# rust-av/grav1synth

Measured on AMD Instinct MI355X. Metric: diff Mpixels/s (luma pixels of frame pairs fully processed: flat-block finder + AR accumulation + block stats + ordered fold), higher is better.
Workload: dtype i8 x i8 -> i32 matrix-core products, i64 sums (exact integers) + f64 flat-block features

## Files before the change

### grav1synth_amd/csrc/engine.hip

```cpp
#include <hip/hip_runtime.h>

#include <algorithm>
#include <chrono>
#include <cmath>
#include <cstdio>
#include <cstring>
#include <atomic>
#include <condition_variable>
#include <deque>
#include <functional>
#include <map>
#include <mutex>
#include <string>
#include <thread>
#include <type_traits>
#include <utility>
#include <vector>

#include "../../include/g1s_diff.h"
#include "fold.h"
#include "frame_op.h"
#include "host_pool.h"
#include "kernels.hip.h"
#include "k1f.hip.h"
// ... 660 lines not shown
    rc = flush_pending();
    if (rc) return rc;
  }
  {
    std::unique_lock<std::mutex> lk(dm);
    cur = (si + 1) % kSlots;
    cv_free.wait(lk, [&] { return !slot_busy[cur]; });
  }
  trace_host("next slot free", cur);
  return G1S_OK;
}

int g1s_diff::plan_batch(int si) {
  Slot &sl = slots[si];
  BatchPlan &p = sl.plan;
  p.g = batch_geom(sl);
  p.wide = wide_ok(p.g, batch_far(sl));
  p.timed = timing;
  p.chain = timing && timing_chain;
  const g1s_sched::Schedule s = g1s_sched::schedule(switches(), {p.timed, device_latest, p.wide, batch, si, p.g.nplanes, last_back});
  if ((s.latest == Role::latest || s.latest == Role::latest2) && !ensure_latest_streams(ss)) return fail_hip("the device half's streams could not be created");
  const hipStream_t of[] = {ss.compute, ss.flat, ss.flat2, ss.copy, ss.upload, ss.latest, ss.latest2};
  p.table = of[(int)s.table], p.finder = of[(int)s.finder], p.accum = of[(int)s.accum], p.rest = of[(int)s.rest];
  p.latest = of[(int)s.latest], p.d2h = of[(int)s.d2h];
  p.back_now = s.back_now, p.after = s.after, p.host_waits = s.host_waits;
  sl.marks.n = 0, sl.marks.timed = p.timed && !p.chain, sl.marks.trace = trace && !p.timed;
  return G1S_OK;
}

int g1s_diff::flush_pending() {
  if (pending < 0) return G1S_OK;
  const int si = pending;
  pending = -1;
  return launch_back(si);
}

int g1s_diff::launch_front(int si) {
  Slot &sl = slots[si];
  const BatchPlan &p = sl.plan;
  const Geom &g = p.g;
  const uint32_t B = sl.count;
  const hipStream_t up = p.table, fstream = p.finder;
  const FrameTable ft{sl.d_planes};
  if (sl.async_in) {
    if (up != ss.upload) {
      if (!h2d_order) HIP_TRY(hipEventCreateWithFlags(&h2d_order.p, hipEventDisableTiming));
      HIP_TRY(hipEventRecord(h2d_order, ss.upload));
      HIP_TRY(hipStreamWaitEvent(up, h2d_order, 0));
    }
    sl.async_in = false;
  }
  sl.marks.mark_trace(up, "table H2D");
  HIP_TRY(hipMemcpyAsync(sl.d_planes, sl.h_planes, sizeof(FramePlanes) * B, hipMemcpyHostToDevice, up));
  sl.marks.mark_trace(up, "k_zero");
  {
    ZeroJob z{};
    int nz = 0;
    auto fill = [&](uint8_t *base, size_t off, size_t bytes) { z.ptr[nz] = reinterpret_cast<uint32_t *>(base + off), z.ndw[nz++] = (uint32_t)(bytes / 4); };
    fill(sl.d_records, 0, L.size * B);
    fill(sl.d_mu, lay.mu_count, lay.mu_only - lay.mu_count);
    fill(sl.d_mu, lay.mu_only, lay.mu_only_bytes);
    fill(sl.d_k1, lay.k1_count, lay.k1 - lay.k1_count);
    if (switches().wide && sl.d_wu) fill(sl.d_wu, lay.wu_lbad, lay.wu_lbad_bytes);
    hipLaunchKernelGGL(k_zero, dim3(256), dim3(256), 0, up, z);
  }
  sl.marks.mark_trace(up, nullptr);
  if (up != p.accum) {
    HIP_TRY(hipEventRecord(ss.table_done[si], up));
    HIP_TRY(hipStreamWaitEvent(p.accum, ss.table_done[si], 0));
    HIP_TRY(hipStreamWaitEvent(fstream, ss.table_done[si], 0));
  }
  if (p.after >= 0) HIP_TRY(hipStreamWaitEvent(fstream, ss.kernels_done[p.after], 0));
  if (p.timed) HIP_TRY(hipEventRecord(sl.ev[kEvStart], fstream));
  {
    const int literal_mode = flat_literal ? flat_literal : switches().k1_literal;
    const int force_literal = literal_mode ? 1 : 0;
    int32_t *mom = reinterpret_cast<int32_t *>(sl.d_k1 + lay.k1_moments);
    CertifyLists cl;
    cl.list = reinterpret_cast<uint32_t *>(sl.d_k1 + lay.k1_list);
    cl.count = reinterpret_cast<uint32_t *>(sl.d_k1 + lay.k1_count);
    cl.global = literal_mode == 0 ? 1 : 0;
    const char *k1_rows = getenv("G1S_K1_ROWS");
    const bool strips = g.fast_rows && g.W % kBlock == 0 && literal_mode == 0 && !(k1_rows && atoi(k1_rows) != 0);
    if (strips) {
      constexpr int kR2 = G1S_STRIP_ROWS2, kRif = G1S_STRIP_RIF;
      constexpr bool kNt = G1S_STRIP_NT != 0, kFold = G1S_STRIP_FOLD != 0;
      if (p.timed && !p.chain) HIP_TRY(hipEventRecord(sl.ev[kEvMomStart], fstream));
      const char *keep_e = getenv("G1S_K1_KEEP_MB");
      const size_t keep_bytes = (size_t)(keep_e ? std::max(atoi(keep_e), 0) : kStripKeepMB) << 20;
      const size_t keep = std::min<size_t>(keep_bytes / ((size_t)g.W * g.src_bps * g.H), B);
      const int nt_frames = kNt ? (int)(B - keep) : 0;
      const dim3 sg((strip_tiles<kR2>(g.nbw, g.nbh) + 3) / 4, B);
      sl.marks.mark(fstream, g.src_bps == 1 ? "k1_moments_strips<1>" : "k1_moments_strips<2>");
      if (g.src_bps == 1)
        hipLaunchKernelGGL((k1_moments_strips<1, kR2, kRif, kNt, kFold>), sg, dim3(256), 0, fstream, ft, g, fc, mom, sl.d_records, sl.d_flags, cl, nt_frames);
      else
        hipLaunchKernelGGL((k1_moments_strips<2, kR2, kRif, kNt, kFold>), sg, dim3(256), 0, fstream, ft, g, fc, mom, sl.d_records, sl.d_flags, cl, nt_frames);
      if (p.timed && !p.chain) HIP_TRY(hipEventRecord(sl.ev[kEvMomEnd], fstream));
    } else {
      if (p.timed && !p.chain) HIP_TRY(hipEventRecord(sl.ev[kEvMomStart], fstream));
      {
        const dim3 mg((g.nblocks + 7) / 8, B);
        sl.marks.mark(fstream, g.src_bps == 1 ? "k1_moments<1>" : "k1_moments<2>");
        if (g.src_bps == 1) hipLaunchKernelGGL(k1_moments<1>, mg, dim3(256), 0, fstream, ft, g, mom);
        else hipLaunchKernelGGL(k1_moments<2>, mg, dim3(256), 0, fstream, ft, g, mom);
      }
      if (p.timed && !p.chain) HIP_TRY(hipEventRecord(sl.ev[kEvMomEnd], fstream));
    }
    if (!strips || !G1S_STRIP_FOLD) {
      sl.marks.mark(fstream, "k1_certify");
      hipLaunchKernelGGL(k1_certify, dim3((g.nblocks + 255) / 256, B), dim3(256), 0, fstream, g, fc, (const int32_t *)mom,
                         sl.d_records, sl.d_flags, cl, force_literal);
    }
    sl.marks.mark(fstream, literal_mode == 1 ? "k1_flat_features" : "k1_flat_block");
    if (literal_mode == 1) {
      dim3 grid((g.nblocks + 63) / 64, B);
      if (g.src_bps == 1)
        hipLaunchKernelGGL((k1_flat_features<1, true>), grid, dim3(64), 0, fstream, ft, g, fc, d_lut, sl.d_records, sl.d_flags,
                           (const uint32_t *)cl.list, (const uint32_t *)cl.count);
      else
        hipLaunchKernelGGL((k1_flat_features<2, true>), grid, dim3(64), 0, fstream, ft, g, fc, d_lut, sl.d_records, sl.d_flags,
                           (const uint32_t *)cl.list, (const uint32_t *)cl.count);
    } else {
      dim3 grid(kFbGrid);
#define G1S_FB(BP, GL) hipLaunchKernelGGL((k1_flat_block<BP, GL>), grid, dim3(64), 0, fstream, ft, g, fc, d_lut, sl.d_records, sl.d_flags, \
                                          (const uint32_t *)cl.list, (const uint32_t *)cl.count, (int)B)
      if (cl.global) {
        if (g.src_bps == 1) G1S_FB(1, true);
        else G1S_FB(2, true);
      } else {
        if (g.src_bps == 1) G1S_FB(1, false);
        else G1S_FB(2, false);
      }
#undef G1S_FB
    }
  }
  if (p.timed && !p.chain) HIP_TRY(hipEventRecord(sl.ev[kEvFinderEnd], fstream));
  const bool w_lists = p.wide;
  WUnitParams wup{};
  if (w_lists) {
    for (int k = 0; k < 2; ++k) {
      wup.units[k] = reinterpret_cast<uint32_t *>(sl.d_wu + lay.wu_units[k]);
      wup.ncell[k] = w_ncell[k];
      wup.gx[k] = w_gx[k];
    }
    wup.count = reinterpret_cast<uint32_t *>(sl.d_wu + lay.wu_count);
    wup.ub[0] = 4;
    wup.ub[1] = w_ub_c;
  }
  sl.marks.mark(fstream, w_lists ? "k2w_select_units" : "k2_flat_select");
  if (w_lists) hipLaunchKernelGGL(k2w_select_units, dim3(B, g.nplanes == 3 ? 2 : 1), dim3(kK2Threads), 0, fstream, g, sl.d_records, (const uint8_t *)sl.d_flags, wup);
  else hipLaunchKernelGGL(k2_flat_select, dim3(B), dim3(kK2Threads), 0, fstream, g, sl.d_records, sl.d_flags);
  if (p.timed && !p.chain) HIP_TRY(hipEventRecord(sl.ev[kEvSelectEnd], fstream));
  if (!w_lists) {
    const MParams mp = make_mparams(sl);
    sl.marks.mark(fstream, "k3m_units");
    hipLaunchKernelGGL(k3m_units, dim3((m_nunits + 255) / 256, B), dim3(256), 0, fstream, g, (const uint8_t *)sl.d_records, mp);
  }
  sl.marks.mark(fstream, nullptr);
  if (fstream != p.accum) HIP_TRY(hipEventRecord(ss.mask_done[si], fstream));
  HIP_TRY(hipGetLastError());
  return G1S_OK;
}

bool g1s_diff::wide_ok(const Geom &g, bool far) const {
  if (!switches().wide || switches().w_off) return false;
  if (g.lag < 1) return false;
  if (wide_gen(g) && !(g.nplanes != 3 || (g.xdec == 1 && g.ydec == 1))) return false;
  const int need = g.nplanes == 3 ? 0x3f : 0x09;
  if ((g.vec_mask & need) != need) return false;
  if (far) return false;
  if ((g.W & 7) != 0 || (g.nplanes == 3 && ((g.W >> g.xdec) & 7) != 0)) return false;
  if (g.nbw > 1023 * 4 || g.nbh > 4095) return false;
  return true;
}

bool g1s_diff::wide_gen(const Geom &g) { return g.src_bps != g.den_bps || g.src_shift != g.den_shift || g.src_shift > 4; }

MParams g1s_diff::make_mparams(const Slot &sl) const {
  MParams mp;
  mp.units = reinterpret_cast<uint32_t *>(sl.d_mu + lay.mu_units);
  mp.unit_count = reinterpret_cast<uint32_t *>(sl.d_mu + lay.mu_count);
  mp.only_any = reinterpret_cast<uint32_t *>(sl.d_mu + lay.mu_any);
  mp.only = sl.d_mu + lay.mu_only;
  mp.partials = sl.d_mpart;
  mp.nunits = m_nunits;
  return mp;
}

int g1s_diff::to_rest(const BatchPlan &p, int si) {
  if (p.rest == p.accum) return G1S_OK;
  HIP_TRY(hipEventRecord(ss.kernels_done[si], p.accum));
  HIP_TRY(hipStreamWaitEvent(p.rest, ss.kernels_done[si], 0));
  return G1S_OK;
}

int g1s_diff::accumulate_wide(Slot &sl, int si) {
  const BatchPlan &p = sl.plan;
// ... 776 lines not shown
```

### grav1synth_amd/csrc/k1f.hip.h

```cpp
#pragma once
#include <hip/hip_runtime.h>
#include <stdint.h>

#include "pixel_helpers.hip.h"
#include "kernels.hip.h"

namespace g1s {

template <int BPS>
__global__ __launch_bounds__(256) void k1_moments(const FrameTable ft, Geom g, int32_t *__restrict__ mom) {
  const int frame = blockIdx.y;
  const int tid = threadIdx.x, yi = tid & 31;
  const int blk = (int)blockIdx.x * 8 + (tid >> 5);
  const bool live = blk < g.nblocks;
  const FramePlanes fp = ft.f[frame];
  const int bx = live ? blk % g.nbw : 0, by = live ? blk / g.nbw : 0;
  const int ox = bx * kBlock, oy = by * kBlock;
  const bool fast = g.fast_rows && (ox + kBlock <= g.W);
  uint32_t pk[8];
  load_row32<BPS>(fp.src[0], fp.src_stride[0], g.src_shift, ox, min(oy + yi, g.H - 1), g.W, fast, pk);
  uint32_t pu[8], pd[8];
#pragma unroll
  for (int k = 0; k < 8; ++k) {
    pu[k] = (uint32_t)__builtin_amdgcn_mov_dpp((int)pk[k], 0x138, 0xf, 0xf, true);
// ... 22 lines not shown
  v16[15] = 0;
  int x[4];
  half_sums_split16(v16, x);
  if (live && yi >= kBlock - 4) {
    int32_t *out = mom + ((size_t)frame * g.nblocks + blk) * kMomInts;
    const int c = yi & 3;
#pragma unroll
    for (int j = 0; j < 4; ++j) out[4 * j + c] = x[j];
  }
}

struct VE {
  double v, e;
};
constexpr double kU = 1.1102230246251565e-16;
__device__ __forceinline__ VE ve_add(VE a, VE b) {
  const double v = a.v + b.v;
  return VE{v, a.e + b.e + 2.0 * kU * fabs(v)};
}
__device__ __forceinline__ VE ve_sub(VE a, VE b) {
  const double v = a.v - b.v;
  return VE{v, a.e + b.e + 2.0 * kU * fabs(v)};
}
__device__ __forceinline__ VE ve_mul(VE a, VE b) {
  const double v = a.v * b.v;
  return VE{v, fabs(a.v) * b.e + fabs(b.v) * a.e + a.e * b.e + 2.0 * kU * fabs(v)};
}
__device__ __forceinline__ VE ve_mul_c(double c, VE a) {
  const double v = c * a.v;
  return VE{v, fabs(c) * a.e + 2.0 * kU * fabs(v)};
}
__device__ __forceinline__ VE ve_div_c(VE a, double c) {
  const double rc = 1.0 / c;
  const double v = a.v * rc;
  return VE{v, a.e * fabs(rc) * (1.0 + 4.0 * kU) + 4.0 * kU * fabs(v)};
}
__device__ __forceinline__ VE ve_add_c(VE a, double c) {
  const double v = a.v + c;
  return VE{v, a.e + 2.0 * kU * fabs(v)};
}
__device__ __forceinline__ int ve_lt(VE a, double K) { return a.v + a.e < K ? 1 : (a.v - a.e >= K ? 0 : -1); }
__device__ __forceinline__ int ve_gt(VE a, double K) { return a.v - a.e > K ? 1 : (a.v + a.e <= K ? 0 : -1); }

struct PE {
  double v, e;
};
__device__ __forceinline__ PE pe_add(PE a, PE b) {
  const double v = a.v + b.v;
  return PE{v, __builtin_fma(2.0 * kU, fabs(v), a.e + b.e)};
}
__device__ __forceinline__ PE pe_sub(PE a, PE b) {
  const double v = a.v - b.v;
  return PE{v, __builtin_fma(2.0 * kU, fabs(v), a.e + b.e)};
}
__device__ __forceinline__ PE pe_mul(PE a, PE b) {
  const double v = a.v * b.v;
  return PE{v, __builtin_fma(2.0 * kU, fabs(v), __builtin_fma(fabs(a.v), b.e, __builtin_fma(fabs(b.v), a.e, a.e * b.e)))};
}
__device__ __forceinline__ PE pe_mul_k(PE a, double k) {
  const double v = a.v * k;
  return PE{v, __builtin_fma(2.0 * kU, fabs(v), fabs(k) * a.e)};
}
__device__ __forceinline__ PE pe_mul_r(PE a, double rc) {
  const double v = a.v * rc;
  return PE{v, __builtin_fma(4.0 * kU, fabs(v), rc * a.e)};
}

__device__ __forceinline__ double sqrt_up(double z) {
  return __builtin_fma((double)__builtin_amdgcn_sqrtf((float)z), 1.0 + 1e-6, 1.1e-19);
}
__device__ __forceinline__ double sqrt_down(double z) {
  return (double)__builtin_amdgcn_sqrtf((float)z) * (1.0 - 1e-6);
}
__device__ __forceinline__ double rcp_up(double d) {
  return (double)__builtin_amdgcn_rcpf((float)d) * (1.0 + 1e-6);
}

struct CertifyLists {
  uint32_t *list;
  uint32_t *count;
  int global;
};

__device__ __forceinline__ void certify_block(const Geom &g, const FlatConsts &fc, const int32_t (&m)[kMomInts], const int frame,
                                              const int blk, const bool live, uint8_t *__restrict__ records,
                                              uint8_t *__restrict__ flags, const CertifyLists &cl, const int force_literal) {
  bool certain = false;
  float score_out = 0.0f;
  uint8_t flag_out = 0;
  if (live && !force_literal) {
    const double S0 = m[kM_S0], SX = (double)m[kM_SXU] - 16.0 * m[kM_S0], SY = (double)m[kM_SYU] - 16.0 * m[kM_S0];
    const double SAX = m[kM_SAX], SAY = m[kM_SAY];
    const double I0 = m[kM_I0], IX = (double)m[kM_IXU] - 16.0 * m[kM_I0], IY = (double)m[kM_IYU] - 16.0 * m[kM_I0];
    const double IPP = m[kM_IPP], DXX = m[kM_DXX], DYY = m[kM_DYY], DXY = m[kM_DXY], DX = m[kM_DX], DY = m[kM_DY];
    const double N = 900.0;
    constexpr double kEt01 = 1030.0 * kU / 4080.0 * (1.0 + 1e-12), kEt2 = 1026.0 * kU / 255.0 * (1.0 + 1e-12);
    const double Et0 = kEt01 * SAY, Et1 = kEt01 * SAX, Et2 = kEt2 * S0;
    double v[5], x[5], cv[3], cx[3], tv[3], tx[3];
    {
      const PE t0 = pe_mul_r(PE{SY, 0.0}, 1.0 / 4080.0), t1 = pe_mul_r(PE{SX, 0.0}, 1.0 / 4080.0), t2 = pe_mul_r(PE{S0, 0.0}, 1.0 / 255.0);
      PE c[3];
#pragma unroll
      for (int i = 0; i < 3; ++i)
        c[i] = pe_add(pe_add(pe_mul_k(t0, fc.ata_inv[3 * i]), pe_mul_k(t1, fc.ata_inv[3 * i + 1])), pe_mul_k(t2, fc.ata_inv[3 * i + 2]));
      const PE c0 = c[0], c1 = c[1], c2 = c[2];
      const PE c00 = pe_mul(c0, c0), c11 = pe_mul(c1, c1), c01 = pe_mul(c0, c1), c0p1 = pe_add(c0, c1);
      const PE sGxx = pe_add(pe_sub(pe_mul_r(PE{DXX, 0.0}, 1.0 / 260100.0), pe_mul_r(pe_mul_k(c1, DX), 1.0 / 4080.0)), pe_mul_k(c11, N / 256.0));
      const PE sGyy = pe_add(pe_sub(pe_mul_r(PE{DYY, 0.0}, 1.0 / 260100.0), pe_mul_r(pe_mul_k(c0, DY), 1.0 / 4080.0)), pe_mul_k(c00, N / 256.0));
      const PE sGxy = pe_add(pe_sub(pe_mul_r(PE{DXY, 0.0}, 1.0 / 260100.0), pe_mul_r(pe_mul_k(c0, DX), 1.0 / 8160.0)),
                             pe_sub(pe_mul_k(c01, N / 256.0), pe_mul_r(pe_mul_k(c1, DY), 1.0 / 8160.0)));
      const PE sR = pe_sub(pe_add(pe_mul_r(PE{I0, 0.0}, 1.0 / 255.0), pe_mul_k(c0p1, 450.0 / 16.0)), pe_mul_k(c2, N));
      const PE cross = pe_add(pe_add(pe_mul_r(pe_mul_k(c0, IY), 1.0 / 4080.0), pe_mul_r(pe_mul_k(c1, IX), 1.0 / 4080.0)),
                              pe_mul_r(pe_mul_k(c2, I0), 1.0 / 255.0));
      const PE fit2 = pe_add(pe_add(pe_mul_k(pe_add(c00, c11), 67650.0 / 256.0), pe_mul_k(pe_mul(c2, c2), N)),
                             pe_sub(pe_mul_k(c01, 450.0 / 256.0), pe_mul_k(pe_mul(c0p1, c2), 900.0 / 16.0)));
      const PE sR2 = pe_add(pe_sub(pe_mul_r(PE{IPP, 0.0}, 1.0 / 65025.0), pe_mul_k(cross, 2.0)), fit2);
      constexpr double kInfl = 1.0 + 1e-7;
      v[0] = sGxx.v, v[1] = sGyy.v, v[2] = sGxy.v, v[3] = sR.v, v[4] = sR2.v;
      x[0] = sGxx.e * kInfl, x[1] = sGyy.e * kInfl, x[2] = sGxy.e * kInfl, x[3] = sR.e * kInfl, x[4] = sR2.e * kInfl;
      cv[0] = c0.v, cv[1] = c1.v, cv[2] = c2.v, cx[0] = c0.e * kInfl, cx[1] = c1.e * kInfl, cx[2] = c2.e * kInfl;
      tv[0] = t0.v, tv[1] = t1.v, tv[2] = t2.v, tx[0] = t0.e * kInfl, tx[1] = t1.e * kInfl, tx[2] = t2.e * kInfl;
    }
    {
      double Ec[3];
#pragma unroll
      for (int i = 0; i < 3; ++i) {
        const double m0 = fc.ata_inv[3 * i], m1 = fc.ata_inv[3 * i + 1], m2 = fc.ata_inv[3 * i + 2];
        Ec[i] = fabs(m0) * (Et0 + 4.0 * kU * (fabs(tv[0]) + tx[0])) + fabs(m1) * (Et1 + 4.0 * kU * (fabs(tv[1]) + tx[1])) +
                fabs(m2) * (Et2 + 4.0 * kU * (fabs(tv[2]) + tx[2]));
      }
      const double F = (fabs(cv[0]) + cx[0]) + (fabs(cv[1]) + cx[1]) + (fabs(cv[2]) + cx[2]) + Ec[0] + Ec[1] + Ec[2];
      const double Eg0 = kU * (3.0 + 5.0 * F);
      const double Egx = Ec[1] / 16.0 + Eg0, Egy = Ec[0] / 16.0 + Eg0;
      const double Er = kU * (2.0 + 5.0 * F) + Ec[0] + Ec[1] + Ec[2];
      const double gxx = fmax(v[0] + x[0], 0.0), gyy = fmax(v[1] + x[1], 0.0), r2 = fmax(v[4] + x[4], 0.0);
      const double kSafety = 4.0;
      const double sxx = sqrt_up(N * gxx), syy = sqrt_up(N * gyy), sr2 = sqrt_up(N * r2);
      VE Gxx{v[0], kSafety * (905.0 * kU * gxx + 2.0 * Egx * sxx + N * Egx * Egx) + x[0]};
      VE Gyy{v[1], kSafety * (905.0 * kU * gyy + 2.0 * Egy * syy + N * Egy * Egy) + x[1]};
      VE Gxy{v[2], kSafety * (905.0 * kU * 0.5 * (gxx + gyy) + Egy * sxx + Egx * syy + N * Egx * Egy) + x[2]};
      VE mean{v[3], kSafety * (905.0 * kU * sr2 + N * (kU * (2.0 + 5.0 * F) + Ec[2] + (Ec[0] + Ec[1]) / 32.0)) + x[3]};
      VE var{v[4], kSafety * (905.0 * kU * r2 + 2.0 * Er * sr2 + N * Er * Er) + x[4]};
      mean = ve_div_c(mean, N);
      Gxx = ve_div_c(Gxx, N);
      Gxy = ve_div_c(Gxy, N);
      Gyy = ve_div_c(Gyy, N);
      var = ve_sub(ve_div_c(var, N), ve_mul(mean, mean));
      const VE trace = ve_add(Gxx, Gyy);
      const VE det = ve_sub(ve_mul(Gxx, Gyy), ve_mul(Gxy, Gxy));
      VE disc = ve_sub(ve_mul(trace, trace), ve_mul_c(4.0, det));
      if (!(disc.v > 0.0)) disc.v = 0.0;
      VE sq;
      sq.v = sqrt(disc.v);
      {
        const double lo = disc.v - disc.e;
        const bool big = lo > disc.e;
        sq.e = (big ? disc.e * rcp_up(2.0 * sqrt_down(lo)) : sqrt_up(disc.e)) + 2.0 * kU * sq.v;
      }
      const VE e1 = ve_div_c(ve_add(trace, sq), 2.0);
      const VE e2 = ve_div_c(ve_sub(trace, sq), 2.0);
      const VE norm = e1;
      VE den = e2;
      if (!(den.v > 1e-6)) den.v = 1e-6;
      VE ratio{e1.v / den.v, 0.0};
      const double den_lo = den.v - den.e;
      const bool ratio_ok = den_lo > 0.0;
      ratio.e = ratio_ok ? (e1.e + fabs(ratio.v) * den.e) * rcp_up(den_lo) * (1.0 + 8.0 * kU) + 2.0 * kU * fabs(ratio.v) : 1e300;
      const double kTrace = 0.15 / 1024.0, kRatio = 1.25, kNorm = 0.08 / 1024.0, kVar = 0.005 / 1024.0;
      const int tr_lt = ve_lt(trace, kTrace), ra_lt = ve_lt(ratio, kRatio), no_lt = ve_lt(norm, kNorm), va_gt = ve_gt(var, kVar);
      int flat;
      if (tr_lt == 0 || ra_lt == 0 || no_lt == 0 || va_gt == 0) flat = 0;
      else if (tr_lt == 1 && ra_lt == 1 && no_lt == 1 && va_gt == 1) flat = 1;
      else flat = -1;
      VE sw = ve_mul_c(-6682.0, var);
      sw = ve_add(sw, ve_mul_c(-0.2056, ratio));
      sw = ve_add(sw, ve_mul_c(13087.0, trace));
      sw = ve_add(sw, ve_mul_c(-12434.0, norm));
      sw = ve_add_c(sw, 2.5694);
      auto clamp_sw = [](double z) { return z < -25.0 ? -25.0 : (z > 100.0 ? 100.0 : z); };
      auto sigmoid = [](double z) { return 1.0 / (1.0 + exp(-z)); };
      const double sv = sigmoid(clamp_sw(sw.v));
      const double x_c = clamp_sw(sw.v);
      const double e_c = fmax(clamp_sw(sw.v + sw.e) - x_c, x_c - clamp_sw(sw.v - sw.e)) * (1.0 + 4.0 * kU);
      const double s_dev = e_c * (sv * (1.0 - sv) + 0.1 * e_c + 8.0 * kU) * (1.0 + 8.0 * kU);
      const double s_lo = sv - s_dev, s_hi = sv + s_dev;
      const float f_lo = (float)(s_lo * (1.0 - 16.0 * kU)), f_hi = (float)(s_hi * (1.0 + 16.0 * kU));
      const bool score_ok = ratio_ok && (f_lo == f_hi) && isfinite(sw.e);
      if (flat >= 0 && va_gt >= 0 && (va_gt == 0 || score_ok)) {
        certain = true;
        flag_out = flat ? 255 : 0;
        score_out = va_gt ? f_lo : 0.0f;
      }
    }
  }
  if (live) {
    uint8_t *rec = records + (size_t)frame * g.rec_size;
    reinterpret_cast<uint32_t *>(rec + g.off_luma_sum)[blk] = (uint32_t)m[kM_CLIP];
    if (certain) {
      reinterpret_cast<float *>(rec + g.off_scores)[blk] = score_out;
      flags[(size_t)frame * g.nblocks + blk] = flag_out;
    }
  }
  const bool todo = live && !certain;
  const unsigned long long bal = __ballot(todo);
  if (bal != 0) {
    const int lane = threadIdx.x & 63;
    uint32_t base = 0;
    if (lane == 0) base = atomicAdd(&cl.count[cl.global ? 0 : frame], (uint32_t)__popcll(bal));
    base = __shfl(base, 0, 64);
    const uint32_t at = base + (uint32_t)__popcll(bal & ((1ull << lane) - 1ull));
    if (todo) {
      if (cl.global) cl.list[at] = (uint32_t)frame * (uint32_t)g.nblocks + (uint32_t)blk;
      else cl.list[(size_t)frame * g.nblocks + at] = (uint32_t)blk;
    }
  }
}

__global__ __launch_bounds__(256) void k1_certify(Geom g, FlatConsts fc, const int32_t *__restrict__ mom,
                                                  uint8_t *__restrict__ records, uint8_t *__restrict__ flags,
                                                  CertifyLists cl, int force_literal) {
  const int frame = blockIdx.y;
  const int blk = (int)blockIdx.x * 256 + (int)threadIdx.x;
  const bool live = blk < g.nblocks;
  int32_t m[kMomInts];
#pragma unroll
  for (int k = 0; k < kMomInts; ++k) m[k] = live ? mom[((size_t)frame * g.nblocks + blk) * kMomInts + k] : 0;
  certify_block(g, fc, m, frame, blk, live, records, flags, cl, force_literal);
}

#ifndef G1S_STRIP_ROWS2
#define G1S_STRIP_ROWS2 0
#endif
#ifndef G1S_STRIP_RIF
#define G1S_STRIP_RIF 4
#endif
#ifndef G1S_STRIP_NT
#define G1S_STRIP_NT 1
#endif
#ifndef G1S_STRIP_FOLD
#define G1S_STRIP_FOLD 1
#endif
constexpr int kStripWgBlocks = 64;
constexpr int kStripKeepMB = 256;
template <int ROWS2>
__host__ __device__ __forceinline__ int strip_tiles_x(int nbw) { return ROWS2 ? (nbw + 7) / 8 : (nbw + 15) / 16; }
template <int ROWS2>
__host__ __device__ __forceinline__ int strip_tiles(int nbw, int nbh) { return strip_tiles_x<ROWS2>(nbw) * (ROWS2 ? (nbh + 1) / 2 : nbh); }
template <int ROWS2>
__device__ __forceinline__ void strip_block_of(int tile, int q, int nbw, int &bx, int &by) {
  const int nx = strip_tiles_x<ROWS2>(nbw);
  const int tx = tile % nx, ty = tile / nx;
  bx = ROWS2 ? tx * 8 + (q & 7) : tx * 16 + q;
  by = ROWS2 ? ty * 2 + (q >> 3) : ty;
}
template <int BPS, bool NT>
__device__ __forceinline__ u32x4 strip_load(gptr_u8 p) {
  if constexpr (BPS == 2) {
    return NT ? __builtin_nontemporal_load((gptr_u4)p) : *(gptr_u4)p;
  } else {
    const u32x2 v = NT ? __builtin_nontemporal_load((gptr_u2)p) : *(gptr_u2)p;
    return u32x4{v.x, v.y, 0u, 0u};
  }
}
template <int BPS>
__device__ __forceinline__ void strip_narrow(const u32x4 raw, int shift, uint32_t (&pk)[2]) {
  if constexpr (BPS == 2) {
    pk[0] = __builtin_amdgcn_perm(raw.y >> shift, raw.x >> shift, 0x06040200u);
    pk[1] = __builtin_amdgcn_perm(raw.w >> shift, raw.z >> shift, 0x06040200u);
  } else {
    pk[0] = raw.x;
    pk[1] = raw.y;
  }
}

template <int BPS, int RIF, bool NT, class RowPtr>
__device__ __forceinline__ void strip_walk(const RowPtr &row_ptr, const int shift, const StripLane &L, StripSums &a) {
  u32x4 raw[RIF];
#pragma unroll
  for (int k = 0; k < RIF; ++k) raw[k] = strip_load<BPS, NT>(row_ptr(k));
  uint32_t pu[2] = {0u, 0u}, pui[2] = {0u, 0u}, pk[2], pd[2] = {0u, 0u}, pi[2];
  strip_narrow<BPS>(raw[0], shift, pk);
  raw[0] = strip_load<BPS, NT>(row_ptr(RIF));
#pragma unroll
  for (int yi = 0; yi < kBlock; ++yi) {
    if (yi + 1 < kBlock) {
      strip_narrow<BPS>(raw[(yi + 1) % RIF], shift, pd);
      if (yi + 1 + RIF < kBlock) raw[(yi + 1) % RIF] = strip_load<BPS, NT>(row_ptr(yi + 1 + RIF));
    }
    strip_row(L, yi, pu, pui, pk, pd, pi, a);
#pragma unroll
    for (int k = 0; k < 2; ++k) pu[k] = pk[k], pui[k] = pi[k], pk[k] = pd[k];
  }
}

template <int BPS, int ROWS2, int RIF, bool NT, bool FOLD>
__global__ __launch_bounds__(256) void k1_moments_strips(const FrameTable ft, Geom g, FlatConsts fc, int32_t *__restrict__ mom,
                                                         uint8_t *__restrict__ records, uint8_t *__restrict__ flags,
                                                         CertifyLists cl, int nt_frames) {
  __shared__ int32_t park[kStripWgBlocks * kMomInts];
  const int frame = blockIdx.y;
  const int lane = (int)(threadIdx.x & 63), c = lane & 3;
  const int wave = __builtin_amdgcn_readfirstlane((int)(threadIdx.x >> 6));
  const int ntiles = strip_tiles<ROWS2>(g.nbw, g.nbh);
  const int tile = (int)blockIdx.x * 4 + wave;
  if (tile < ntiles) {
    int bx, by;
    strip_block_of<ROWS2>(tile, lane >> 2, g.nbw, bx, by);
    const bool live = bx < g.nbw && by < g.nbh;
    if (!live) bx = 0, by = 0;
    const FramePlanes fp = ft.f[frame];
    const uint32_t stride = fp.src_stride[0];
    const int shift = g.src_shift;
    const int oy = ROWS2 ? by * kBlock : (tile / strip_tiles_x<ROWS2>(g.nbw)) * kBlock;
    const uint32_t xoff = (uint32_t)(bx * kBlock + c * 8) * BPS;
    auto row_ptr = [&](int yi) {
      const uintptr_t row = (uintptr_t)fp.src[0] + (size_t)min(oy + yi, g.H - 1) * stride;
      if constexpr (ROWS2) return (gptr_u8)row + xoff;
      else
        return (gptr_u8)(((uintptr_t)(uint32_t)__builtin_amdgcn_readfirstlane((int)(row >> 32)) << 32) |
                         (uint32_t)__builtin_amdgcn_readfirstlane((int)(uint32_t)row)) + xoff;
    };
    const StripLane L = strip_lane(c);
    StripSums a{};
    if (NT && frame < nt_frames) strip_walk<BPS, RIF, true>(row_ptr, shift, L, a);
    else strip_walk<BPS, RIF, false>(row_ptr, shift, L, a);
    int v16[16], x[4];
    strip_totals(a, c, max(oy + kBlock - g.H, 0), v16);
    quad_sums_split16(v16, x);
    if constexpr (FOLD) {
      int32_t *out = park + (wave * 16 + (lane >> 2)) * kMomInts;
#pragma unroll
      for (int j = 0; j < 4; ++j) out[4 * j + c] = x[j];
    } else if (live) {
      int32_t *out = mom + ((size_t)frame * g.nblocks + (by * g.nbw + bx)) * kMomInts;
#pragma unroll
      for (int j = 0; j < 4; ++j) out[4 * j + c] = x[j];
    }
  }
  if constexpr (FOLD) {
    __syncthreads();
    if (wave != 0) return;
    const int t = (int)blockIdx.x * 4 + (lane >> 4);
    int bx, by;
    strip_block_of<ROWS2>(t, lane & 15, g.nbw, bx, by);
    const bool live = t < ntiles && bx < g.nbw && by < g.nbh;
    int32_t m[kMomInts];
#pragma unroll
    for (int k = 0; k < kMomInts; ++k) m[k] = live ? park[lane * kMomInts + k] : 0;
    certify_block(g, fc, m, frame, live ? by * g.nbw + bx : 0, live, records, flags, cl, 0);
  }
}

}
```

### grav1synth_amd/csrc/kernels.hip.h

```cpp
#pragma once
#include <hip/hip_runtime.h>
#include <stdint.h>

#include "record.h"

namespace g1s {

struct FramePlanes {
  const uint8_t *src[3];
  const uint8_t *den[3];
  uint32_t src_stride[3];
  uint32_t den_stride[3];
};

constexpr int kMaxBatch = 256;
struct FrameTable {
  const FramePlanes *f;
};

struct Geom {
  int W, H, xdec, ydec, nplanes;
  int nbw, nbh, nblocks;
  int src_bps, den_bps, src_shift, den_shift;
  int lag, n;
// ... 175 lines not shown
    for (int y0 = 0; y0 < kBlock; y0 += 4) {
      if (y0 + 4 < kBlock) {
#pragma unroll
        for (int k = 0; k < 4; ++k) load_row_raw<BPS>(base, stride, ox, min(oy + y0 + 4 + k, g.H - 1), rb4[k]);
      }
#pragma unroll
      for (int k = 0; k < 4; ++k) {
        uint32_t pk[8];
        narrow_row<BPS>(ra4[k], shift, pk);
        fit_row(y0 + k, pk);
      }
#pragma unroll
      for (int k = 0; k < 4; ++k) ra4[k] = rb4[k];
    }
  } else {
    for (int yi = 0; yi < kBlock; ++yi) {
      uint32_t pk[8];
      load_row32<BPS>(base, stride, shift, ox, min(oy + yi, g.H - 1), g.W, false, pk);
      fit_row(yi, pk);
    }
  }
  double c0 = 0.0, c1 = 0.0, c2 = 0.0;
  c0 += fc.ata_inv[0] * t0; c0 += fc.ata_inv[1] * t1; c0 += fc.ata_inv[2] * t2;
  c1 += fc.ata_inv[3] * t0; c1 += fc.ata_inv[4] * t1; c1 += fc.ata_inv[5] * t2;
  c2 += fc.ata_inv[6] * t0; c2 += fc.ata_inv[7] * t1; c2 += fc.ata_inv[8] * t2;

  double ra[kBlock], rb[kBlock];
  RowRaw<BPS> nxt;
  if (fast) load_row_raw<BPS>(base, stride, ox, min(oy, g.H - 1), nxt);
  auto take_row = [&](int yi, uint32_t (&pk)[8]) {
    if (fast) {
      const RowRaw<BPS> cur = nxt;
      if (yi + 1 < kBlock) load_row_raw<BPS>(base, stride, ox, min(oy + yi + 1, g.H - 1), nxt);
      narrow_row<BPS>(cur, shift, pk);
    } else {
      load_row32<BPS>(base, stride, shift, ox, min(oy + yi, g.H - 1), g.W, false, pk);
    }
  };
  auto resid_row = [&](int yi, double (&out)[kBlock]) {
    uint32_t pk[8];
    take_row(yi, pk);
    const double yc = 0.0 + ((double)(yi - 16) * 0.0625) * c0;
#pragma unroll
    for (int xi = 0; xi < kBlock; ++xi) {
      const double xd = (double)(xi - 16) * 0.0625;
      const double fit = (yc + xd * c1) + c2;
      out[xi] = lut[(pk[xi >> 2] >> (8 * (xi & 3))) & 0xffu] - fit;
    }
  };
  double Gxx = 0.0, Gxy = 0.0, Gyy = 0.0, var = 0.0, mean = 0.0;
  auto grad_row = [&](int yi, double (&up)[kBlock], const double (&cur)[kBlock]) {
    uint32_t pk[8];
    take_row(yi + 1, pk);
    const double yc = 0.0 + ((double)(yi + 1 - 16) * 0.0625) * c0;
#pragma unroll
    for (int xi = 0; xi < kBlock; ++xi) {
      const double xd = (double)(xi - 16) * 0.0625;
      const double fit = (yc + xd * c1) + c2;
      const double nv = lut[(pk[xi >> 2] >> (8 * (xi & 3))) & 0xffu] - fit;
      if (xi >= 1 && xi <= kBlock - 2) {
        const double gx = (cur[xi + 1] - cur[xi - 1]) * 0.5;
        const double gy = (nv - up[xi]) * 0.5;
        Gxx += gx * gx;
        Gxy += gx * gy;
        Gyy += gy * gy;
        mean += cur[xi];
        var += cur[xi] * cur[xi];
      }
      up[xi] = nv;
    }
  };
  resid_row(0, ra);
  resid_row(1, rb);
  for (int yi = 1; yi < kBlock - 1; yi += 2) {
    grad_row(yi, ra, rb);
    grad_row(yi + 1, rb, ra);
  }

  flat_decide(Gxx, Gxy, Gyy, var, mean, g, records, flags, frame, blk);
}

constexpr int kFbGrid = 768;
constexpr int kFbInner = (kBlock - 2) * (kBlock - 2);
template <int BPS, bool GLOBAL>
__global__ __launch_bounds__(64) void k1_flat_block(const FrameTable ft, Geom g, FlatConsts fc,
                                                    const double *__restrict__ lut_g, uint8_t *__restrict__ records,
                                                    uint8_t *__restrict__ flags, const uint32_t *__restrict__ list,
                                                    const uint32_t *__restrict__ count, int nframes) {
  __shared__ double lut[256];
  __shared__ double s_v[kBlock * kBlock];
  __shared__ double s_t[5 * kFbInner];
  __shared__ uint32_t s_pre[GLOBAL ? 1 : kMaxBatch + 1];
  const int lane = threadIdx.x;
  const int W = (int)gridDim.x, w = (int)blockIdx.x;
  int total;
  if (GLOBAL) {
    total = (int)count[0];
    if (w >= total) return;
    for (int i = lane; i < 256; i += 64) lut[i] = lut_g[i];
  } else {
    uint32_t carry = 0;
    if (lane == 0) s_pre[0] = 0;
    for (int base = 0; base < nframes; base += 64) {
      const uint32_t c = base + lane < nframes ? count[base + lane] : 0u;
      uint32_t incl = c;
#pragma unroll
      for (int o = 1; o < 64; o <<= 1) {
        const uint32_t t = (uint32_t)__shfl_up((int)incl, o, 64);
        if (lane >= o) incl += t;
      }
      if (base + lane < nframes) s_pre[base + lane + 1] = carry + incl;
      carry += (uint32_t)__shfl((int)incl, 63, 64);
    }
    __syncthreads();
    total = (int)s_pre[nframes];
  }
  bool have_lut = GLOBAL;
  int frame = 0;
  for (int p = w; p < total; p += W) {
  int blk;
  if (GLOBAL) {
    const uint32_t e = list[p];
    frame = (int)(e / (uint32_t)g.nblocks);
    blk = (int)(e - (uint32_t)frame * (uint32_t)g.nblocks);
  } else {
    while ((int)s_pre[frame + 1] <= p) ++frame;
    blk = (int)list[(size_t)frame * g.nblocks + (p - (int)s_pre[frame])];
  }
  if (!have_lut) {
    for (int i = lane; i < 256; i += 64) lut[i] = lut_g[i];
    have_lut = true;
  }
  const FramePlanes fp = ft.f[frame];
  {
    const int bx = blk % g.nbw, by = blk / g.nbw;
    const int ox = bx * kBlock, oy = by * kBlock;
    __syncthreads();
    int pxs[kBlock * kBlock / 64];
#pragma unroll
    for (int k = 0; k < kBlock * kBlock / 64; ++k) {
      const int i = lane + 64 * k, yi = i >> 5, xi = i & 31;
      pxs[k] = load_px<BPS>(fp.src[0], fp.src_stride[0], g.src_shift, min(ox + xi, g.W - 1), min(oy + yi, g.H - 1));
    }
#pragma unroll
    for (int k = 0; k < kBlock * kBlock / 64; ++k) {
      const int i = lane + 64 * k, yi = i >> 5, xi = i & 31;
      const double v = lut[pxs[k]];
      const double yd = (double)(yi - 16) * 0.0625, xd = (double)(xi - 16) * 0.0625;
      s_v[i] = v;
      s_t[i] = v * yd;
      s_t[kBlock * kBlock + i] = v * xd;
      s_t[2 * kBlock * kBlock + i] = v;
    }
    __syncthreads();
    double sum = 0.0;
    if (lane < 3) {
      const double *src = s_t + lane * (kBlock * kBlock);
#pragma unroll 16
      for (int i = 0; i < kBlock * kBlock; ++i) sum += src[i];
    }
    const double t0 = __shfl(sum, 0, 64), t1 = __shfl(sum, 1, 64), t2 = __shfl(sum, 2, 64);
    double c0 = 0.0, c1 = 0.0, c2 = 0.0;
    c0 += fc.ata_inv[0] * t0; c0 += fc.ata_inv[1] * t1; c0 += fc.ata_inv[2] * t2;
    c1 += fc.ata_inv[3] * t0; c1 += fc.ata_inv[4] * t1; c1 += fc.ata_inv[5] * t2;
    c2 += fc.ata_inv[6] * t0; c2 += fc.ata_inv[7] * t1; c2 += fc.ata_inv[8] * t2;
    __syncthreads();
#pragma unroll 4
    for (int i = lane; i < kBlock * kBlock; i += 64) {
      const int yi = i >> 5, xi = i & 31;
      const double yc = 0.0 + ((double)(yi - 16) * 0.0625) * c0;
      const double xd = (double)(xi - 16) * 0.0625;
      const double fit = (yc + xd * c1) + c2;
      s_v[i] = s_v[i] - fit;
    }
    __syncthreads();
    for (int j = lane; j < kFbInner; j += 64) {
      const int yi = 1 + j / (kBlock - 2), xi = 1 + j % (kBlock - 2);
      const int o = yi * kBlock + xi;
      const double cur = s_v[o];
      const double gx = (s_v[o + 1] - s_v[o - 1]) * 0.5;
      const double gy = (s_v[o + kBlock] - s_v[o - kBlock]) * 0.5;
      s_t[j] = gx * gx;
      s_t[kFbInner + j] = gx * gy;
      s_t[2 * kFbInner + j] = gy * gy;
      s_t[3 * kFbInner + j] = cur;
      s_t[4 * kFbInner + j] = cur * cur;
    }
    __syncthreads();
    sum = 0.0;
    if (lane < 5) {
      const double *src = s_t + lane * kFbInner;
#pragma unroll 12
      for (int j = 0; j < kFbInner; ++j) sum += src[j];
    }
    const double Gxx = __shfl(sum, 0, 64), Gxy = __shfl(sum, 1, 64), Gyy = __shfl(sum, 2, 64);
    const double mean = __shfl(sum, 3, 64), var = __shfl(sum, 4, 64);
    if (lane == 0) flat_decide(Gxx, Gxy, Gyy, var, mean, g, records, flags, frame, blk);
  }
  }
}

constexpr int kK2Threads = 1024;
constexpr int kK2PerThread = 8;
__device__ __forceinline__ uint32_t wave_scan_incl(uint32_t v) {
  int x = (int)v;
  x += __builtin_amdgcn_update_dpp(0, x, 0x111, 0xf, 0xf, false);
  x += __builtin_amdgcn_update_dpp(0, x, 0x112, 0xf, 0xf, false);
  x += __builtin_amdgcn_update_dpp(0, x, 0x114, 0xf, 0xf, false);
  x += __builtin_amdgcn_update_dpp(0, x, 0x118, 0xf, 0xf, false);
  x += __builtin_amdgcn_update_dpp(0, x, 0x142, 0xa, 0xf, false);
  x += __builtin_amdgcn_update_dpp(0, x, 0x143, 0xc, 0xf, false);
  return (uint32_t)x;
}

template <int PER>
__device__ __forceinline__ void k2_flat_select_sized(const Geom &g, uint8_t *__restrict__ records, const uint8_t *__restrict__ flags, int frame,
                                                     uint32_t *lds_bits) {
  __shared__ __attribute__((aligned(16))) uint32_t s_hist[3][256];
  uint8_t *rec = records + (size_t)frame * g.rec_size;
  const uint32_t *sc = reinterpret_cast<const uint32_t *>(rec + g.off_scores);
  const int nb = g.nblocks;
  const int tid = threadIdx.x, lane = tid & 63;
  const bool in_regs = nb <= kK2Threads * PER;
  const uint8_t *fl = flags + (size_t)frame * nb;
  uint32_t v[PER];
#pragma unroll
  for (int k = 0; k < PER; ++k) {
    const int i = tid + k * kK2Threads;
    v[k] = i < nb ? sc[i] : 0xffffffffu;
  }
  constexpr bool kEarlyFlags = PER <= 8;
  uint8_t f[PER];
  if (kEarlyFlags && in_regs) {
#pragma unroll
    for (int k = 0; k < PER; ++k) {
      const int i = tid + k * kK2Threads;
      f[k] = i < nb ? fl[i] : 0;
    }
  }
  if (tid < 256) s_hist[0][tid] = 0;
  __syncthreads();
  uint32_t rank = (uint32_t)(nb * 90 / 100);
  uint32_t thr = 0;
  for (int pass = 0; pass < 4; ++pass) {
    const int shift = 24 - 8 * pass;
    const uint32_t himask = pass ? ~0u << (shift + 8) : 0u;
    uint32_t *hist = s_hist[pass % 3];
    if (tid < 256) s_hist[(pass + 1) % 3][tid] = 0;
    if (in_regs && pass == 0) {
#pragma unroll
      for (int k = 0; k < PER; ++k) {
        const uint32_t d = v[k] >> 24;
        unsigned long long todo = __ballot(1);
        while (todo) {
          const int first = __ffsll((long long)todo) - 1;
          const uint32_t dv = (uint32_t)__shfl((int)d, first, 64);
          const unsigned long long same = __ballot(d == dv) & todo;
          if (lane == first) atomicAdd(&hist[dv], (uint32_t)__popcll(same));
          todo &= ~same;
        }
      }
    } else if (in_regs && PER > 8) {
#pragma unroll
      for (int k = 0; k < PER; ++k) {
        const bool in = (v[k] & himask) == thr;
        const uint32_t d = (v[k] >> shift) & 0xffu;
        unsigned long long todo = __ballot(in);
#pragma unroll
        for (int r = 0; r < 2; ++r) {
          if (!todo) break;
          const int first = __ffsll((long long)todo) - 1;
          const uint32_t dv = (uint32_t)__shfl((int)d, first, 64);
          const unsigned long long same = __ballot(in && d == dv) & todo;
          if (lane == first) atomicAdd(&hist[dv], (uint32_t)__popcll(same));
          todo &= ~same;
        }
        if ((todo >> lane) & 1ull) atomicAdd(&hist[d], 1u);
      }
    } else if (in_regs) {
#pragma unroll
      for (int k = 0; k < PER; ++k)
// ... 228 lines not shown
```

Baseline: 664,900.

## Fuse literal flat-block fallback into strip moments kernel, dropping separate launch

The strip moments kernel now handles the uncertified blocks in place. Each workgroup ballots which of its blocks could not be certified, then runs the full literal flat-block computation for them with all four waves, reusing LDS that is re-aliased between the park buffer and the term arrays. This removes the separate k1_flat_block launch and its global work list. In exchange the strip kernel needs more LDS, and workgroups with many uncertain blocks become serial hotspots, which could lower occupancy and unbalance the load.

New measurement: 665,800, median of 6. No clear change (+0.1%).

```diff
diff --git a/grav1synth_amd/csrc/engine.hip b/grav1synth_amd/csrc/engine.hip
--- a/grav1synth_amd/csrc/engine.hip
+++ b/grav1synth_amd/csrc/engine.hip
@@ -766,9 +766,12 @@
     cl.global = literal_mode == 0 ? 1 : 0;
     const char *k1_rows = getenv("G1S_K1_ROWS");
     const bool strips = g.fast_rows && g.W % kBlock == 0 && literal_mode == 0 && !(k1_rows && atoi(k1_rows) != 0);
+    constexpr bool kStripLit = G1S_STRIP_FOLD != 0 && G1S_STRIP_LITERAL != 0;
     if (strips) {
       constexpr int kR2 = G1S_STRIP_ROWS2, kRif = G1S_STRIP_RIF;
       constexpr bool kNt = G1S_STRIP_NT != 0, kFold = G1S_STRIP_FOLD != 0;
+      const char *all_open_e = getenv("G1S_K1_STRIPS_LITERAL");
+      const int all_open = kStripLit && all_open_e && atoi(all_open_e) != 0 ? 1 : 0;
       if (p.timed && !p.chain) HIP_TRY(hipEventRecord(sl.ev[kEvMomStart], fstream));
       const char *keep_e = getenv("G1S_K1_KEEP_MB");
       const size_t keep_bytes = (size_t)(keep_e ? std::max(atoi(keep_e), 0) : kStripKeepMB) << 20;
@@ -777,9 +780,11 @@
       const dim3 sg((strip_tiles<kR2>(g.nbw, g.nbh) + 3) / 4, B);
       sl.marks.mark(fstream, g.src_bps == 1 ? "k1_moments_strips<1>" : "k1_moments_strips<2>");
       if (g.src_bps == 1)
-        hipLaunchKernelGGL((k1_moments_strips<1, kR2, kRif, kNt, kFold>), sg, dim3(256), 0, fstream, ft, g, fc, mom, sl.d_records, sl.d_flags, cl, nt_frames);
+        hipLaunchKernelGGL((k1_moments_strips<1, kR2, kRif, kNt, kFold, kStripLit>), sg, dim3(256), 0, fstream, ft, g, fc, mom, sl.d_records, sl.d_flags, cl,
+                           nt_frames, (const double *)d_lut, all_open);
       else
-        hipLaunchKernelGGL((k1_moments_strips<2, kR2, kRif, kNt, kFold>), sg, dim3(256), 0, fstream, ft, g, fc, mom, sl.d_records, sl.d_flags, cl, nt_frames);
+        hipLaunchKernelGGL((k1_moments_strips<2, kR2, kRif, kNt, kFold, kStripLit>), sg, dim3(256), 0, fstream, ft, g, fc, mom, sl.d_records, sl.d_flags, cl,
+                           nt_frames, (const double *)d_lut, all_open);
       if (p.timed && !p.chain) HIP_TRY(hipEventRecord(sl.ev[kEvMomEnd], fstream));
     } else {
       if (p.timed && !p.chain) HIP_TRY(hipEventRecord(sl.ev[kEvMomStart], fstream));
@@ -796,8 +801,10 @@
       hipLaunchKernelGGL(k1_certify, dim3((g.nblocks + 255) / 256, B), dim3(256), 0, fstream, g, fc, (const int32_t *)mom,
                          sl.d_records, sl.d_flags, cl, force_literal);
     }
-    sl.marks.mark(fstream, literal_mode == 1 ? "k1_flat_features" : "k1_flat_block");
-    if (literal_mode == 1) {
+    const bool tail = !(strips && kStripLit);
+    if (tail) sl.marks.mark(fstream, literal_mode == 1 ? "k1_flat_features" : "k1_flat_block");
+    if (!tail) {
+    } else if (literal_mode == 1) {
       dim3 grid((g.nblocks + 63) / 64, B);
       if (g.src_bps == 1)
         hipLaunchKernelGGL((k1_flat_features<1, true>), grid, dim3(64), 0, fstream, ft, g, fc, d_lut, sl.d_records, sl.d_flags,
diff --git a/grav1synth_amd/csrc/k1f.hip.h b/grav1synth_amd/csrc/k1f.hip.h
--- a/grav1synth_amd/csrc/k1f.hip.h
+++ b/grav1synth_amd/csrc/k1f.hip.h
@@ -128,7 +128,8 @@
   int global;
 };
 
-__device__ __forceinline__ void certify_block(const Geom &g, const FlatConsts &fc, const int32_t (&m)[kMomInts], const int frame,
+template <bool APPEND = true>
+__device__ __forceinline__ bool certify_block(const Geom &g, const FlatConsts &fc, const int32_t (&m)[kMomInts], const int frame,
                                               const int blk, const bool live, uint8_t *__restrict__ records,
                                               uint8_t *__restrict__ flags, const CertifyLists &cl, const int force_literal) {
   bool certain = false;
@@ -248,18 +249,21 @@
     }
   }
   const bool todo = live && !certain;
-  const unsigned long long bal = __ballot(todo);
-  if (bal != 0) {
-    const int lane = threadIdx.x & 63;
-    uint32_t base = 0;
-    if (lane == 0) base = atomicAdd(&cl.count[cl.global ? 0 : frame], (uint32_t)__popcll(bal));
-    base = __shfl(base, 0, 64);
-    const uint32_t at = base + (uint32_t)__popcll(bal & ((1ull << lane) - 1ull));
-    if (todo) {
-      if (cl.global) cl.list[at] = (uint32_t)frame * (uint32_t)g.nblocks + (uint32_t)blk;
-      else cl.list[(size_t)frame * g.nblocks + at] = (uint32_t)blk;
-    }
-  }
+  if constexpr (APPEND) {
+    const unsigned long long bal = __ballot(todo);
+    if (bal != 0) {
+      const int lane = threadIdx.x & 63;
+      uint32_t base = 0;
+      if (lane == 0) base = atomicAdd(&cl.count[cl.global ? 0 : frame], (uint32_t)__popcll(bal));
+      base = __shfl(base, 0, 64);
+      const uint32_t at = base + (uint32_t)__popcll(bal & ((1ull << lane) - 1ull));
+      if (todo) {
+        if (cl.global) cl.list[at] = (uint32_t)frame * (uint32_t)g.nblocks + (uint32_t)blk;
+        else cl.list[(size_t)frame * g.nblocks + at] = (uint32_t)blk;
+      }
+    }
+  }
+  return todo;
 }
 
 __global__ __launch_bounds__(256) void k1_certify(Geom g, FlatConsts fc, const int32_t *__restrict__ mom,
@@ -285,6 +289,9 @@
 #endif
 #ifndef G1S_STRIP_FOLD
 #define G1S_STRIP_FOLD 1
+#endif
+#ifndef G1S_STRIP_LITERAL
+#define G1S_STRIP_LITERAL 1
 #endif
 constexpr int kStripWgBlocks = 64;
 constexpr int kStripKeepMB = 256;
@@ -339,11 +346,16 @@
   }
 }
 
-template <int BPS, int ROWS2, int RIF, bool NT, bool FOLD>
+template <int BPS, int ROWS2, int RIF, bool NT, bool FOLD, bool LIT>
 __global__ __launch_bounds__(256) void k1_moments_strips(const FrameTable ft, Geom g, FlatConsts fc, int32_t *__restrict__ mom,
                                                          uint8_t *__restrict__ records, uint8_t *__restrict__ flags,
-                                                         CertifyLists cl, int nt_frames) {
-  __shared__ int32_t park[kStripWgBlocks * kMomInts];
+                                                         CertifyLists cl, int nt_frames, const double *__restrict__ lut_g,
+                                                         int all_open) {
+  constexpr bool kLit = FOLD && LIT;
+  constexpr int kParkBytes = kStripWgBlocks * kMomInts * 4;
+  constexpr int kLitDoubles = kBlock * kBlock + kFbTermDoubles + kFbSumDoubles + 1;
+  __shared__ __attribute__((aligned(16))) unsigned char lds[kLit ? kLitDoubles * 8 : kParkBytes];
+  int32_t *const park = reinterpret_cast<int32_t *>(lds + (kLit ? kBlock * kBlock * 8 : 0));
   const int frame = blockIdx.y;
   const int lane = (int)(threadIdx.x & 63), c = lane & 3;
   const int wave = __builtin_amdgcn_readfirstlane((int)(threadIdx.x >> 6));
@@ -385,16 +397,44 @@
   }
   if constexpr (FOLD) {
     __syncthreads();
-    if (wave != 0) return;
-    const int t = (int)blockIdx.x * 4 + (lane >> 4);
-    int bx, by;
-    strip_block_of<ROWS2>(t, lane & 15, g.nbw, bx, by);
-    const bool live = t < ntiles && bx < g.nbw && by < g.nbh;
-    int32_t m[kMomInts];
-#pragma unroll
-    for (int k = 0; k < kMomInts; ++k) m[k] = live ? park[lane * kMomInts + k] : 0;
-    certify_block(g, fc, m, frame, live ? by * g.nbw + bx : 0, live, records, flags, cl, 0);
-  }
-}
-
-}
+    if (!kLit && wave != 0) return;
+    bool todo = false;
+    if (wave == 0) {
+      const int t = (int)blockIdx.x * 4 + (lane >> 4);
+      int bx, by;
+      strip_block_of<ROWS2>(t, lane & 15, g.nbw, bx, by);
+      const bool live = t < ntiles && bx < g.nbw && by < g.nbh;
+      int32_t m[kMomInts];
+#pragma unroll
+      for (int k = 0; k < kMomInts; ++k) m[k] = live ? park[lane * kMomInts + k] : 0;
+      todo = certify_block<!kLit>(g, fc, m, frame, live ? by * g.nbw + bx : 0, live, records, flags, cl, kLit ? all_open : 0);
+    }
+    if constexpr (kLit) {
+      static_assert(kFbTermDoubles * 8 >= kParkBytes, "park lies over the term arrays");
+      double *const s_v = reinterpret_cast<double *>(lds), *const s_t = s_v + kBlock * kBlock, *const s_r = s_t + kFbTermDoubles;
+      uint32_t *const s_open = reinterpret_cast<uint32_t *>(s_r + kFbSumDoubles);
+      if (wave == 0) {
+        const unsigned long long bal = __ballot(todo);
+        if (lane == 0) {
+          s_open[0] = (uint32_t)bal, s_open[1] = (uint32_t)(bal >> 32);
+          if (bal != 0) atomicAdd(&cl.count[0], (uint32_t)__popcll(bal));
+        }
+      }
+      __syncthreads();
+      unsigned long long open = ((unsigned long long)(uint32_t)__builtin_amdgcn_readfirstlane((int)s_open[1]) << 32) |
+                                (uint32_t)__builtin_amdgcn_readfirstlane((int)s_open[0]);
+      if (open == 0) return;
+      const FramePlanes fp = ft.f[frame];
+      const G1S_GLOBAL double *const lut = (const G1S_GLOBAL double *)(uintptr_t)lut_g;
+      while (open != 0) {
+        const int q = __builtin_ctzll(open);
+        open &= open - 1;
+        int bx, by;
+        strip_block_of<ROWS2>((int)blockIdx.x * 4 + (q >> 4), q & 15, g.nbw, bx, by);
+        literal_block<BPS, 4>(fp, g, fc, lut, records, flags, frame, by * g.nbw + bx, (int)threadIdx.x, s_v, s_t, s_r);
+      }
+    }
+  }
+}
+
+}
diff --git a/grav1synth_amd/csrc/kernels.hip.h b/grav1synth_amd/csrc/kernels.hip.h
--- a/grav1synth_amd/csrc/kernels.hip.h
+++ b/grav1synth_amd/csrc/kernels.hip.h
@@ -281,14 +281,93 @@
 
 constexpr int kFbGrid = 768;
 constexpr int kFbInner = (kBlock - 2) * (kBlock - 2);
+constexpr int kFbTermDoubles = 4 * kFbInner;
+constexpr int kFbSumDoubles = 8;
+template <int BPS, int NW, class LutPtr>
+__device__ __forceinline__ void literal_block(const FramePlanes &fp, const Geom &g, const FlatConsts &fc, const LutPtr lut,
+                                              uint8_t *__restrict__ records, uint8_t *__restrict__ flags, const int frame,
+                                              const int blk, const int tid, double *__restrict__ s_v, double *__restrict__ s_t,
+                                              double *__restrict__ s_r) {
+  constexpr int kT = 64 * NW, kPer = kBlock * kBlock / kT;
+  static_assert(kPer * kT == kBlock * kBlock, "the workgroup's threads divide the block");
+  const int bx = blk % g.nbw, by = blk / g.nbw;
+  const int ox = bx * kBlock, oy = by * kBlock;
+  const bool work = tid < kT;
+  __syncthreads();
+  if (work) {
+    int pxs[kPer];
+#pragma unroll
+    for (int k = 0; k < kPer; ++k) {
+      const int i = tid + kT * k, yi = i >> 5, xi = i & 31;
+      pxs[k] = load_px<BPS>(fp.src[0], fp.src_stride[0], g.src_shift, min(ox + xi, g.W - 1), min(oy + yi, g.H - 1));
+    }
+#pragma unroll
+    for (int k = 0; k < kPer; ++k) {
+      const int i = tid + kT * k, yi = i >> 5, xi = i & 31;
+      const double v = lut[pxs[k]];
+      const double yd = (double)(yi - 16) * 0.0625, xd = (double)(xi - 16) * 0.0625;
+      s_v[i] = v;
+      s_t[i] = v * yd;
+      s_t[kBlock * kBlock + i] = v * xd;
+    }
+  }
+  __syncthreads();
+  if (tid < 3) {
+    const double *src = tid == 2 ? s_v : s_t + tid * (kBlock * kBlock);
+    double sum = 0.0;
+#pragma unroll 16
+    for (int i = 0; i < kBlock * kBlock; ++i) sum += src[i];
+    s_r[tid] = sum;
+  }
+  __syncthreads();
+  const double t0 = s_r[0], t1 = s_r[1], t2 = s_r[2];
+  double c0 = 0.0, c1 = 0.0, c2 = 0.0;
+  c0 += fc.ata_inv[0] * t0; c0 += fc.ata_inv[1] * t1; c0 += fc.ata_inv[2] * t2;
+  c1 += fc.ata_inv[3] * t0; c1 += fc.ata_inv[4] * t1; c1 += fc.ata_inv[5] * t2;
+  c2 += fc.ata_inv[6] * t0; c2 += fc.ata_inv[7] * t1; c2 += fc.ata_inv[8] * t2;
+#pragma unroll 4
+  for (int i = work ? tid : kBlock * kBlock; i < kBlock * kBlock; i += kT) {
+    const int yi = i >> 5, xi = i & 31;
+    const double yc = 0.0 + ((double)(yi - 16) * 0.0625) * c0;
+    const double xd = (double)(xi - 16) * 0.0625;
+    const double fit = (yc + xd * c1) + c2;
+    s_v[i] = s_v[i] - fit;
+  }
+  __syncthreads();
+  for (int j = work ? tid : kFbInner; j < kFbInner; j += kT) {
+    const int yi = 1 + j / (kBlock - 2), xi = 1 + j % (kBlock - 2);
+    const int o = yi * kBlock + xi;
+    const double cur = s_v[o];
+    const double gx = (s_v[o + 1] - s_v[o - 1]) * 0.5;
+    const double gy = (s_v[o + kBlock] - s_v[o - kBlock]) * 0.5;
+    s_t[j] = gx * gx;
+    s_t[kFbInner + j] = gx * gy;
+    s_t[2 * kFbInner + j] = gy * gy;
+    s_t[3 * kFbInner + j] = cur * cur;
+  }
+  __syncthreads();
+  if (tid < 5) {
+    const double *src = tid == 3 ? s_v + kBlock + 1 : s_t + (tid == 4 ? 3 : tid) * kFbInner;
+    const int pitch = tid == 3 ? kBlock : kBlock - 2;
+    double sum = 0.0;
+    for (int yi = 0; yi < kBlock - 2; ++yi) {
+      const double *row = src + yi * pitch;
+#pragma unroll 15
+      for (int xi = 0; xi < kBlock - 2; ++xi) sum += row[xi];
+    }
+    s_r[tid] = sum;
+  }
+  __syncthreads();
+  if (tid == 0) flat_decide(s_r[0], s_r[1], s_r[2], s_r[4], s_r[3], g, records, flags, frame, blk);
+}
+
 template <int BPS, bool GLOBAL>
 __global__ __launch_bounds__(64) void k1_flat_block(const FrameTable ft, Geom g, FlatConsts fc,
                                                     const double *__restrict__ lut_g, uint8_t *__restrict__ records,
                                                     uint8_t *__restrict__ flags, const uint32_t *__restrict__ list,
                                                     const uint32_t *__restrict__ count, int nframes) {
   __shared__ double lut[256];
-  __shared__ double s_v[kBlock * kBlock];
-  __shared__ double s_t[5 * kFbInner];
+  __shared__ double s_v[kBlock * kBlock], s_t[kFbTermDoubles], s_r[kFbSumDoubles];
   __shared__ uint32_t s_pre[GLOBAL ? 1 : kMaxBatch + 1];
   const int lane = threadIdx.x;
   const int W = (int)gridDim.x, w = (int)blockIdx.x;
@@ -331,71 +410,7 @@
     have_lut = true;
   }
   const FramePlanes fp = ft.f[frame];
-  {
-    const int bx = blk % g.nbw, by = blk / g.nbw;
-    const int ox = bx * kBlock, oy = by * kBlock;
-    __syncthreads();
-    int pxs[kBlock * kBlock / 64];
-#pragma unroll
-    for (int k = 0; k < kBlock * kBlock / 64; ++k) {
-      const int i = lane + 64 * k, yi = i >> 5, xi = i & 31;
-      pxs[k] = load_px<BPS>(fp.src[0], fp.src_stride[0], g.src_shift, min(ox + xi, g.W - 1), min(oy + yi, g.H - 1));
-    }
-#pragma unroll
-    for (int k = 0; k < kBlock * kBlock / 64; ++k) {
-      const int i = lane + 64 * k, yi = i >> 5, xi = i & 31;
-      const double v = lut[pxs[k]];
-      const double yd = (double)(yi - 16) * 0.0625, xd = (double)(xi - 16) * 0.0625;
-      s_v[i] = v;
-      s_t[i] = v * yd;
-      s_t[kBlock * kBlock + i] = v * xd;
-      s_t[2 * kBlock * kBlock + i] = v;
-    }
-    __syncthreads();
-    double sum = 0.0;
-    if (lane < 3) {
-      const double *src = s_t + lane * (kBlock * kBlock);
-#pragma unroll 16
-      for (int i = 0; i < kBlock * kBlock; ++i) sum += src[i];
-    }
-    const double t0 = __shfl(sum, 0, 64), t1 = __shfl(sum, 1, 64), t2 = __shfl(sum, 2, 64);
-    double c0 = 0.0, c1 = 0.0, c2 = 0.0;
-    c0 += fc.ata_inv[0] * t0; c0 += fc.ata_inv[1] * t1; c0 += fc.ata_inv[2] * t2;
-    c1 += fc.ata_inv[3] * t0; c1 += fc.ata_inv[4] * t1; c1 += fc.ata_inv[5] * t2;
-    c2 += fc.ata_inv[6] * t0; c2 += fc.ata_inv[7] * t1; c2 += fc.ata_inv[8] * t2;
-    __syncthreads();
-#pragma unroll 4
-    for (int i = lane; i < kBlock * kBlock; i += 64) {
-      const int yi = i >> 5, xi = i & 31;
-      const double yc = 0.0 + ((double)(yi - 16) * 0.0625) * c0;
-      const double xd = (double)(xi - 16) * 0.0625;
-      const double fit = (yc + xd * c1) + c2;
-      s_v[i] = s_v[i] - fit;
-    }
-    __syncthreads();
-    for (int j = lane; j < kFbInner; j += 64) {
-      const int yi = 1 + j / (kBlock - 2), xi = 1 + j % (kBlock - 2);
-      const int o = yi * kBlock + xi;
-      const double cur = s_v[o];
-      const double gx = (s_v[o + 1] - s_v[o - 1]) * 0.5;
-      const double gy = (s_v[o + kBlock] - s_v[o - kBlock]) * 0.5;
-      s_t[j] = gx * gx;
-      s_t[kFbInner + j] = gx * gy;
-      s_t[2 * kFbInner + j] = gy * gy;
-      s_t[3 * kFbInner + j] = cur;
-      s_t[4 * kFbInner + j] = cur * cur;
-    }
-    __syncthreads();
-    sum = 0.0;
-    if (lane < 5) {
-      const double *src = s_t + lane * kFbInner;
-#pragma unroll 12
-      for (int j = 0; j < kFbInner; ++j) sum += src[j];
-    }
-    const double Gxx = __shfl(sum, 0, 64), Gxy = __shfl(sum, 1, 64), Gyy = __shfl(sum, 2, 64);
-    const double mean = __shfl(sum, 3, 64), var = __shfl(sum, 4, 64);
-    if (lane == 0) flat_decide(Gxx, Gxy, Gyy, var, mean, g, records, flags, frame, blk);
-  }
+  literal_block<BPS, 1>(fp, g, fc, (const double *)lut, records, flags, frame, blk, lane, s_v, s_t, s_r);
   }
 }
 
```
